# BarclayII/audiogan

Measured on AMD Instinct MI355X. Metric: audio-samples/sec per G+D train step (8 kHz, 8192-sample clips), higher is better.
Workload: dtype f32; 1 GPU; C2: full audiogan.py Conv1d/LSTM G + D, batch 64 per GPU, 8192-sample white-noise clips, frame_size 256 (T=32), canonical G+D step, adam, per-parameter clip d=1 g=0.1; global_batch=64, clip_len=8192, parallelism=dp1, launch=hipGraph replay (1 graph per step)

## Files before the change

### audiogan_amd/_lib.py

```python
import ctypes as C
import os

_HERE = os.path.dirname(os.path.abspath(__file__))
LIB_PATH = os.path.join(_HERE, 'libaudiogan_hip.so')

AG_OK, AG_ERR_ARG, AG_ERR_LAUNCH, AG_ERR_UNSUPPORTED = 0, -1, -2, -3
ACT_NONE, ACT_LEAKY, ACT_TANH, ACT_LEAKY_GATE = 0, 1, 2, 3
OPT_RMSPROP, OPT_ADAM = 0, 1
FLAG_NAN, FLAG_BIG = 1, 2

vp, i32, i64, f32 = C.c_void_p, C.c_int32, C.c_int64, C.c_float


class WnDesc(C.Structure):
    _fields_ = [('v', vp), ('g', vp), ('w', vp), ('wpa', vp), ('wpb', vp), ('inv_norm', vp),
                ('rows', i32), ('cols', i32), ('d1', i32), ('K', i32), ('stride', i32), ('pad_', i32)]


class WnBwdDesc(C.Structure):
    _fields_ = [('v', vp), ('g', vp), ('dw', vp), ('dv', vp), ('dg', vp), ('rows', i32), ('cols', i32),
                ('accumulate', i32), ('pad_', i32)]


class ConvArgs(C.Structure):
# ... 26 lines not shown
    'ag_arch': (C.c_char_p, []),
    'ag_last_error': (C.c_char_p, []),
    'ag_last_kernel': (C.c_char_p, []),
    'ag_weight_norm_fwd': (C.c_int, [vp, C.c_int, C.c_int, vp]),
    'ag_weight_norm_bwd': (C.c_int, [vp, C.c_int, C.c_int, vp]),
    'ag_conv1d_engine': (C.c_int, [C.POINTER(ConvArgs), vp]),
    'ag_prep_conv_weight': (C.c_int, [vp, vp, vp, C.c_int, C.c_int, C.c_int, C.c_int, C.c_int, vp]),
    'ag_wpa_numel': (i64, [C.c_int, C.c_int, C.c_int]),
    'ag_wpb_numel': (i64, [C.c_int, C.c_int, C.c_int, C.c_int]),
    'ag_conv1d_wgrad': (C.c_int, [vp, i64, i64, vp, i64, i64, vp] + [C.c_int] * 8 + [vp]),
    'ag_conv1d_o1_fwd': (C.c_int, [vp, i64, i64, vp, vp, vp, i64, C.c_int, C.c_int, C.c_int, C.c_int, C.c_int,
                                   C.c_int, f32, vp]),
    'ag_conv1d_o1_bwd_data': (C.c_int, [vp, i64, vp, vp, i64, i64, C.c_int, C.c_int, C.c_int, C.c_int, C.c_int,
                                        C.c_int, vp]),
    'ag_conv1d_o1_wgrad': (C.c_int, [vp, i64, vp, i64, i64, vp, C.c_int, C.c_int, C.c_int, C.c_int, C.c_int, vp]),
    'ag_channel_sum': (C.c_int, [vp, i64, i64, vp, C.c_int, C.c_int, C.c_int, C.c_int, vp]),
    'ag_lstm_front_bwd_step': (C.c_int, [vp, C.c_int, vp, C.c_int, vp, C.c_int, C.c_int, vp, vp, C.c_int, vp, vp, vp,
                                         vp, vp, vp, C.c_int, C.c_int, vp]),
    'ag_leaky_bwd': (C.c_int, [vp, i64, i64, vp, i64, i64, vp, i64, i64, vp, i64, i64, vp, vp, C.c_int,
                               C.c_int, C.c_int, f32, vp]),
    'ag_gemm': (C.c_int, [vp, C.c_int, C.c_int, vp, C.c_int, C.c_int, vp, C.c_int, C.c_int,
                          C.c_int, C.c_int, f32, f32, vp, vp, C.c_int, C.c_int, f32, vp]),
    'ag_col_sum': (C.c_int, [vp, C.c_int, C.c_int, vp, C.c_int, C.c_int, C.c_int, vp]),
    'ag_lstm_cell_fwd': (C.c_int, [vp, C.c_int, vp, C.c_int, vp, C.c_int, vp, C.c_int, vp, C.c_int,
                                   vp, C.c_int, vp, C.c_int, C.c_int, C.c_int, vp]),
    'ag_lstm_cell_bwd': (C.c_int, [vp, C.c_int, vp, C.c_int, vp, C.c_int, vp, C.c_int, vp, C.c_int,
                                   vp, C.c_int, vp, C.c_int, vp, C.c_int, vp, C.c_int, vp, C.c_int,
                                   C.c_int, C.c_int, vp]),
    'ag_gru_cell_fwd': (C.c_int, [vp, vp, vp, C.c_int, vp, C.c_int, C.c_int, C.c_int, vp]),
    'ag_gru_cell_bwd': (C.c_int, [vp, vp, vp, C.c_int, vp, C.c_int, vp, vp, vp, C.c_int, C.c_int, C.c_int, vp]),
    'ag_skinny_gemm': (C.c_int, [vp, C.c_int, vp, C.c_int, C.c_int, vp, C.c_int, C.c_int, C.c_int, C.c_int,
                                 f32, vp, C.c_int, f32, C.c_int, vp]),
    'ag_lstm_step_fwd': (C.c_int, [vp, vp, C.c_int, vp, C.c_int, C.c_int, vp, vp, vp, vp, vp, C.c_int,
                                   C.c_int, C.c_int, vp]),
    'ag_lstm_seq_fwd': (C.c_int, [vp, vp, vp, vp, vp, vp, vp, C.c_int, C.c_int, C.c_int, C.c_int, C.c_int, C.c_int, vp]),
    'ag_lstm_seq_bwd': (C.c_int, [vp, vp, vp, vp, vp, vp, vp, vp, C.c_int, C.c_int, C.c_int, C.c_int, C.c_int, C.c_int, C.c_int, vp]),
    'ag_set_precision': (C.c_int, [C.c_int]),
    'ag_get_precision': (C.c_int, []),
    'ag_bind_workspace': (C.c_int, [vp, i64]),
    'ag_conv1d_wgrad_ws_numel': (i64, [C.c_int] * 5),
    'ag_gemm_ws_numel': (i64, [C.c_int] * 4),
    'ag_skinny_ws_numel': (i64, [C.c_int] * 3),
    'ag_persist_debug': (C.c_int, [i64, C.c_int]),
    'ag_lstm_persist_ok': (C.c_int, [C.c_int, C.c_int, C.c_int, C.c_int]),
    'ag_lstm_persist_ws_bytes': (i64, [C.c_int, C.c_int, C.c_int]),
    'ag_lstm_seq_fwd_persist': (C.c_int, [vp, vp, vp, vp, C.c_int, vp, vp, vp, i64, C.c_int, C.c_int, C.c_int, C.c_int, C.c_int, vp]),
# ... 82 lines not shown
```

### audiogan_amd/csrc/gemm.hip

```cpp
#include <cstdlib>
#include <type_traits>

#include "common.h"
#include "gemm_tile.h"

#ifndef GBK
#define GBK 16
#endif
#define GKQ (GBK / 4)


template <int ROWS>
struct KContig {
  static constexpr int ITER = ROWS * (GBK / 4) / 256;
  static_assert(ITER >= 1, "tile too small");
  f32x4 v[ITER];
  __device__ __forceinline__ void load(const float* __restrict__ G, int ld, int r0, int nrows, int k0, int K,
                                       bool vec, int tid) {
#pragma unroll
    for (int it = 0; it < ITER; ++it) {
      const int idx = tid + it * 256;
      const int r = idx / GKQ, kq = idx % GKQ;
      const int gr = r0 + r, gk = k0 + kq * 4;
      f32x4 q = {0.f, 0.f, 0.f, 0.f};
// ... 642 lines not shown
extern "C" int ag_col_sum(const void* X, int x_bf16, int ldx, float* out, int M, int N, int accumulate, void* stream) {
  const AgWs ws = ag_ws_take();
  AG_REQUIRE(X && out && M > 0 && N > 0 && ldx >= N, "ag_col_sum: bad args");
  const int gx = ag_cdiv(N, 64);
  int gy = ag_cdiv(1024, gx);
  if (gy > ag_cdiv(M, 16)) gy = ag_cdiv(M, 16);
  if (gy < 1) gy = 1;
  float* part = nullptr;
  if (gy > 1 && ws.p && ws.numel >= 2 * (int64_t)N) {
    if ((int64_t)gy * N > ws.numel) gy = (int)(ws.numel / N);
    part = ws.p;
  } else {
    gy = 1;
  }
  const int rows_per = ag_cdiv(M, gy);
  gy = ag_cdiv(M, rows_per);
  if (gy == 1) part = nullptr;
  hipLaunchKernelGGL(col_sum_kernel, dim3(gx, gy), dim3(256), 0, (hipStream_t)stream, (const float*)X, ldx, out, M,
                     N, rows_per, part, accumulate, x_bf16 ? 1 : 0);
  AG_CHECK_LAUNCH("ag_col_sum");
  if (part) return ag_slab_reduce(part, gy, N, out, accumulate ? 1 : 0, (hipStream_t)stream);
  return AG_OK;
}
```

### audiogan_amd/csrc/pointwise.hip

```cpp
#include "common.h"

__global__ __launch_bounds__(256) void weight_norm_fwd_kernel(const ag_wn_desc* __restrict__ descs) {
  const ag_wn_desc d = descs[blockIdx.y];
  const int lane = threadIdx.x & 63;
  const int r = blockIdx.x * 4 + (threadIdx.x >> 6);
  if (r >= d.rows) return;
  const float* v = d.v + (int64_t)r * d.cols;
  float ss = 0.f;
  for (int i = lane; i < d.cols; i += 64) {
    const float x = v[i];
    ss += x * x;
  }
  ss = ag_wave_sum(ss);
  const float nrm = sqrtf(ss);
  const float sc = d.g[r] / nrm;
  if (lane == 0 && d.inv_norm) d.inv_norm[r] = 1.f / nrm;
  const int d0p32 = (d.rows + 31) / 32 * 32;
  const int s = d.stride > 0 ? d.stride : 1;
  const int mt = (d.K + s - 1) / s;
  const int mp = (d.d1 * s + 31) / 32 * 32;
  const bool aligned = d.wpb && ag_scatter_aligned(d.K, s, d.pad);
  unsigned short* qa = d.wpa ? reinterpret_cast<unsigned short*>(d.wpa + ag_wq_offset((d.d1 + 1) & ~1, d.K, d0p32)) : nullptr;
  unsigned short* qb = d.wpb ? reinterpret_cast<unsigned short*>(d.wpb + ag_wq_offset((d.rows + 1) & ~1, mt, mp)) : nullptr;
  for (int i = lane; i < d.cols; i += 64) {
// ... 723 lines not shown
      const int64_t o = (int64_t)b * obs + (int64_t)j * ors + i;
      const float v = tile[tx][ty + 8 * k];
      if (OUT16) reinterpret_cast<unsigned short*>(out)[o] = (unsigned short)(ag_pack_bf16(v, v) & 0xFFFFu);
      else reinterpret_cast<float*>(out)[o] = v;
    }
  }
}

extern "C" int ag_transpose_batched(const void* in, int in_bf16, int64_t ibs, int64_t irs, void* out, int out_bf16, int64_t obs,
                                    int64_t ors, int B, int R, int Cc, void* stream) {
  AG_REQUIRE(in && out && B > 0 && R > 0 && Cc > 0 && B <= 65535, "ag_transpose_batched: bad args");
  AG_REQUIRE(irs >= Cc && ors >= R, "ag_transpose_batched: a row pitch is smaller than its row");
  AG_REQUIRE(ag_cdiv(R, 32) <= 65535, "ag_transpose_batched: too many rows");
  const dim3 grid(ag_cdiv(Cc, 32), ag_cdiv(R, 32), B);
  hipStream_t st = (hipStream_t)stream;
  if (!in_bf16 && !out_bf16) hipLaunchKernelGGL((transpose_batched_kernel<false, false>), grid, dim3(256), 0, st, in, ibs, irs, out, obs, ors, R, Cc);
  if (!in_bf16 && out_bf16) hipLaunchKernelGGL((transpose_batched_kernel<false, true>), grid, dim3(256), 0, st, in, ibs, irs, out, obs, ors, R, Cc);
  if (in_bf16 && !out_bf16) hipLaunchKernelGGL((transpose_batched_kernel<true, false>), grid, dim3(256), 0, st, in, ibs, irs, out, obs, ors, R, Cc);
  if (in_bf16 && out_bf16) hipLaunchKernelGGL((transpose_batched_kernel<true, true>), grid, dim3(256), 0, st, in, ibs, irs, out, obs, ors, R, Cc);
  AG_CHECK_LAUNCH("ag_transpose_batched");
  return AG_OK;
}

__global__ __launch_bounds__(256) void build_zc_kernel(const float* __restrict__ z, const float* __restrict__ c,
                                                       float* __restrict__ zc, int B, int T, int ns, int es) {
  const int F = ns + es;
  const int64_t n = (int64_t)T * B * F;
  for (int64_t i = (int64_t)blockIdx.x * 256 + threadIdx.x; i < n; i += (int64_t)gridDim.x * 256) {
    const int j = (int)(i % F);
    const int64_t tb = i / F;
    const int b = (int)(tb % B), t = (int)(tb / B);
    zc[i] = j < ns ? z[((int64_t)b * T + t) * ns + j] : c[(int64_t)b * es + (j - ns)];
  }
}

extern "C" int ag_build_zc(const float* z, const float* c, float* zc, int B, int T, int ns, int es, void* stream) {
  AG_REQUIRE(z && c && zc && B > 0 && T > 0 && ns >= 0 && es >= 0 && ns + es > 0, "ag_build_zc: bad args");
  const int64_t n = (int64_t)T * B * (ns + es);
  int gx = (int)ag_cdiv64(n, 256 * 4);
  if (gx > 4096) gx = 4096;
  hipLaunchKernelGGL(build_zc_kernel, dim3(gx), dim3(256), 0, (hipStream_t)stream, z, c, zc, B, T, ns, es);
  AG_CHECK_LAUNCH("ag_build_zc");
  return AG_OK;
}

struct CriticBatchP {
// ... 312 lines not shown
```

### audiogan_amd/kernels.py

```python
import ctypes as C

import torch

from . import _lib
from ._lib import lib, check, ACT_NONE, ACT_LEAKY, ACT_TANH, ACT_LEAKY_GATE, OPT_RMSPROP, OPT_ADAM

LEAKY_SLOPE = 0.01


def _stream():
    return C.c_void_p(torch.cuda.current_stream().cuda_stream)


def _p(t):
    return C.c_void_p(t.data_ptr()) if t is not None else C.c_void_p(0)


def _chk(t, name, dtype=torch.float32):
    if t is None:
        return
    if not t.is_cuda:
        raise RuntimeError('audiogan_amd: %s must be a CUDA (HIP) tensor; there is no CPU path' % name)
    if t.dtype != dtype:
        raise TypeError('audiogan_amd: %s must be %s, got %s' % (name, dtype, t.dtype))
# ... 375 lines not shown
        check(lib.ag_gemm(_p(A), lda, int(ta), _p(B), ldb, int(tb), _p(Cm), ldc, M, N, K, alpha, beta,
                          _p(bias), _p(res), ldres, act, slope, _stream()), 'ag_gemm')
    finally:
        if hold:
            lib.ag_defer_reduces(3)


def col_sum(X, out, accumulate=True, defer=True):
    ldx = _mat_any(X, 'X')
    _chk(out, 'out')
    M, N = X.shape
    assert out.numel() == N and out.is_contiguous()
    hold = (not defer) and reduces_recording()
    if hold:
        lib.ag_defer_reduces(2)
    try:
        _ws = _bind_ws(min(_SMALL_WS, 64 * N) if M > 16 else 0, out.device)
        check(lib.ag_col_sum(_p(X), int(_is16(X)), ldx, _p(out), M, N, int(bool(accumulate)), _stream()), 'ag_col_sum')
    finally:
        if hold:
            lib.ag_defer_reduces(3)


def lstm_cell_fwd(gates, c_prev, c_out, h_out=None, y_out=None, h_prev=None, valid=None, t=0):
    ldg = _mat(gates, 'gates')
    B, H4 = gates.shape
    H = H4 // 4
    _chk(valid, 'valid', torch.int64)
    ld = lambda x, n: (_mat(x, n) if x is not None else 0)
    for x in (c_prev, c_out, h_out, y_out, h_prev):
        assert x is None or tuple(x.shape) == (B, H)
    check(lib.ag_lstm_cell_fwd(_p(gates), ldg, _p(c_prev), ld(c_prev, 'c_prev'), _p(h_out),
                               ld(h_out, 'h_out'), _p(c_out), ld(c_out, 'c_out'), _p(y_out),
                               ld(y_out, 'y_out'), _p(h_prev), ld(h_prev, 'h_prev'), _p(valid), t, B, H,
                               _stream()), 'ag_lstm_cell_fwd')


def lstm_cell_bwd(gates_act, c_prev, c_new, dh, dy, dc_next, dgates, dc_prev, dh_pass=None,
                  valid=None, t=0):
    B, H4 = gates_act.shape
    H = H4 // 4
    _chk(valid, 'valid', torch.int64)
    ld = lambda x, n: (_mat(x, n) if x is not None else 0)
    for x in (c_prev, c_new, dh, dy, dc_next, dc_prev, dh_pass):
        assert x is None or tuple(x.shape) == (B, H)
    assert tuple(dgates.shape) == (B, H4)
# ... 55 lines not shown


def bct_to_tbc(x, out=None, out_dtype=None):
    _chk_any(x, 'x')
    B, Cc, T = x.shape
    assert x.stride(2) == 1
    if out is None:
        out = torch.empty(T, B, Cc, device=x.device, dtype=out_dtype or x.dtype)
    _chk_any(out, 'out')
    check(lib.ag_transpose_batched(_p(x), int(_is16(x)), x.stride(0), x.stride(1), _p(out), int(_is16(out)), Cc, B * Cc, B, Cc,
                                   T, _stream()), 'ag_transpose_batched')
    return out


def tbc_to_bct(x, out=None, out_dtype=None):
    _chk_any(x, 'x')
    T, B, Cc = x.shape
    assert x.is_contiguous()
    if out is None:
        out = torch.empty(B, Cc, T, device=x.device, dtype=out_dtype or x.dtype)
    _chk_any(out, 'out')
    check(lib.ag_transpose_batched(_p(x), int(_is16(x)), Cc, B * Cc, _p(out), int(_is16(out)), Cc * T, T, B, T, Cc, _stream()),
          'ag_transpose_batched')
    return out


def rowdot_ok(x, w):
    return x.dim() == 2 and x.stride(1) == 1 and w.numel() == x.size(1) and w.is_contiguous()


def rowdot_fwd(x, w, bias, y):
    ldx = _mat_any(x, 'x')
    _chk(w, 'w'); _chk(bias, 'bias'); _chk(y, 'y')
    M, Kd = x.shape
    assert rowdot_ok(x, w) and y.numel() == M
    ldy = y.stride(0) if M > 1 else 1
    check(lib.ag_rowdot_fwd(_p(x), int(_is16(x)), ldx, _p(w), _p(bias), _p(y), ldy, M, Kd, _stream()), 'ag_rowdot_fwd')


def rowdot_bwd(dy, x, w, dx=None, dw=None, db=None, gate=False, slope=LEAKY_SLOPE, accumulate=True):
    ldx = _mat_any(x, 'x')
    _chk(dy, 'dy'); _chk(w, 'w'); _chk_any(dx, 'dx'); _chk(dw, 'dw'); _chk(db, 'db')
    M, Kd = x.shape
    assert rowdot_ok(x, w) and dy.numel() == M
    lddx = _mat_any(dx, 'dx') if dx is not None else 0
    assert dx is None or (tuple(dx.shape) == (M, Kd) and dx.dtype == x.dtype), 'x and dx share a storage type'
# ... 229 lines not shown
        nl = w_[3] if len(w_) > 3 else 1
        only = Profiler.only
        if key is None:
            sig = _call_sig(a, k)
            if only is not None and seen.get(sig, only) != only:
                return fn(*a, **k)
        elif only is not None and key != only:
            return fn(*a, **k)
        e0, e1 = torch.cuda.Event(enable_timing=True), torch.cuda.Event(enable_timing=True)
        e0.record()
        r = fn(*a, **k)
        e1.record()
        if key is None:
            key = seen[sig] = lib.ag_last_kernel().decode()
        Profiler.records.append((key, fl, by, e0, e1, nl))
        return r
    wrapped.__name__ = name
    wrapped.__doc__ = fn.__doc__
    wrapped.__module__ = __name__
    globals()[name] = wrapped


for _n, _w in (('gemm', _work_gemm), ('conv_engine', _work_conv), ('conv_wgrad', _work_wgrad),
               ('channel_sum', None), ('leaky_bwd', None), ('col_sum', None), ('lstm_cell_fwd', None),
               ('lstm_cell_bwd', None), ('weight_norm_fwd', None), ('weight_norm_bwd', None),
               ('bce_logits_fwd', None), ('bce_logits_bwd', None), ('act_fwd', None), ('act_bwd', None),
               ('axpby', None), ('grad_norms', None), ('opt_step', None)):
    _instrument(_n, _w)


def _al16(t):
    return t.data_ptr() % 16 == 0


def skinny_ok(A, B, tb):
    M, Kd = A.shape
    ok = M <= 256 and Kd % 8 == 0 and A.stride(1) == 1 and A.stride(0) % 4 == 0 and _al16(A)
    if tb:
        ok = ok and B.stride(1) == 1 and B.stride(0) % 4 == 0 and _al16(B)
    return ok


def skinny_gemm(A, B, Cm, tb=False, beta=0.0, bias=None, act=ACT_NONE, slope=LEAKY_SLOPE, atomic=False):
    lda, ldb, ldc = _mat(A, 'A'), _mat(B, 'B'), _mat(Cm, 'C')
    M, N = Cm.shape
    Kd = A.size(1)
    assert A.size(0) == M and (B.size(1) if tb else B.size(0)) == Kd and (B.size(0) if tb else B.size(1)) == N
# ... 758 lines not shown
```

### audiogan_amd/modules.py

```python
import torch
import torch.nn as nn

from . import ops
from .common import prepare_groups
from .ops import ConvSpec


def div_roundup(x, d):
    return (x + d - 1) // d


def roundup(x, d):
    return (x + d - 1) // d * d


class Replicated(nn.Module):

    def __init__(self, module):
        super().__init__()
        self.module = module

    def forward(self, *a, **k):
        return self.module(*a, **k)

# ... 252 lines not shown
            _add(self._head.group, r.linear, 'weight')
            _add(self._head.group, r.linear, 'bias')
        for i in (0, 2):
            _add(self._head.group, self.classifier.module[i], 'weight')
            _add(self._head.group, self.classifier.module[i], 'bias')

    def _stride_prods(self, dev):
        t = getattr(self, '_prods', None)
        if t is None or t[0].device != dev:
            p = torch.tensor(list(_cumprod([s for _, s, _ in self.cnn_struct])), device=dev).view(-1, 1)
            t = self._prods = (p, p - 1)
        return t

    def _rnn_weights(self, layer):
        out = []
        for suffix in ('', '_reverse'):
            for n in ('weight_ih', 'weight_hh', 'bias_ih', 'bias_hh'):
                out.append(getattr(self.rnn, '%s_l%d%s' % (n, layer, suffix)))
        return out

    def stride_products(self):
        return list(_cumprod([s for _, s, _ in self.cnn_struct]))

    def features(self, x, length, lens_all=None):
        if lens_all is None:
            length = length.to(x.device).long()
            prods, prods_m1 = self._stride_prods(x.device)
            lens_all = torch.div(length.view(1, -1) + prods_m1, prods, rounding_mode='floor')
        lens_list = [lens_all[i] for i in range(lens_all.size(0))]
        acts = ops.DConvStackFn.apply(x, self._stack, lens_list, *self._stack.group.params())
        return acts, lens_list

    def stores_bf16(self, batch, dev):
        K = ops.K
        dev = torch.device(dev)
        h = self._state_size // 2
        return bool(dev.type == 'cuda' and K.bf16_storage() and K.lstm_step_ok(batch, h) and
                    K.lstm_persist_ok(batch, h, 2, dev) and K.lstm_persist_bwd_ok(batch, h, 2, dev))

    def classify(self, a, n, c):
        ss, es = self._state_size, self._embed_size
        b, tq = a.size(0), a.size(2)
        s16 = self.stores_bf16(b, a.device)
        seq = ops.TimeMajorFn.apply(a, s16)
        for layer in range(self._num_layers):
            seq = ops.LSTMSeqFn.apply(seq, n, 2, c if layer == 0 else None, *self._rnn_weights(layer))
        logits = ops.DHeadFn.apply(seq.reshape(tq * b, ss), self._head, *self._head.group.params())
        return logits.view(tq, b).t()

    def early_params(self):
        conv = set(id(p) for p in self.cnn.parameters())
        return [p for p in self.parameters() if id(p) not in conv]

    def prepare_weights(self):
        prepare_groups([self._stack.group, self._head.group])

    def forward(self, x, length, c, percent_used=0.1, lens_all=None):
        self.prepare_weights()
        acts, lens_list = self.features(x, length, lens_all)
        n = lens_list[-1]
        return self.classify(acts[-1], n, c), list(acts), lens_list, n


class Embedder(nn.Module):

    def __init__(self, output_size=100, char_embed_size=50, num_layers=1, num_chars=256):
        super().__init__()
        self._output_size = output_size
        self._char_embed_size = char_embed_size
        self._num_layers = num_layers
        self.embed = Replicated(nn.Embedding(num_chars, char_embed_size))
        self.rnn = nn.LSTM(char_embed_size, output_size // 2, num_layers, bidirectional=True)

    def forward(self, chars, length):
        nl, b, o = self._num_layers, chars.size(0), self._output_size
        dev = self.embed.module.weight.device
        length = length.to(dev).long()
        seq = self.embed.module.weight[chars.to(dev).long()].permute(1, 0, 2).contiguous()
        for layer in range(nl):
            w = []
            for suffix in ('', '_reverse'):
                for n in ('weight_ih', 'weight_hh', 'bias_ih', 'bias_hh'):
                    w.append(getattr(self.rnn, '%s_l%d%s' % (n, layer, suffix)))
            seq = ops.LSTMSeqFn.apply(seq, length, 2, None, *w)
# ... 24 lines not shown
```

### audiogan_amd/ops.py

```python
import torch

from . import kernels as K
from .kernels import ACT_NONE, ACT_LEAKY, ACT_TANH, ACT_LEAKY_GATE

from .common import PARAM_EPOCH, Prepared, WNGroup, _zeros_like_list


class ConvSpec(object):
    __slots__ = ('kind', 'cin', 'cout', 'K', 'stride', 'pad', 'out_pad')

    def __init__(self, kind, cin, cout, K_, stride, pad, out_pad=0):
        self.kind, self.cin, self.cout, self.K, self.stride, self.pad = kind, cin, cout, K_, stride, pad
        self.out_pad = out_pad

    def out_len(self, lin):
        if self.kind == 'conv':
            return (lin + 2 * self.pad - self.K) // self.stride + 1
        return (lin - 1) * self.stride - 2 * self.pad + self.K + self.out_pad


def _o1(spec):
    return K.conv_o1_ok(spec.kind, spec.cout, spec.K, spec.stride, spec.pad)


# ... 102 lines not shown
            add = dslab[:, cin - ds.cout:cin] if cin >= ds.cout else None
            K.leaky_bwd(dout, out_v, dout, add_into=add, bias_grad=dws[4 * i + 3] if wg else None)
            hid = hids[i]
            if wg:
                conv_wgrad(ds, hid, dout, dws[4 * i + 2], None)
            dhid = torch.empty_like(hid)
            conv_bwd_data(ds, qw, dout, dhid, gate=hid)
            if wg:
                K.channel_sum(dhid, dws[4 * i + 1])
            if wg:
                conv_wgrad(cs, slab[:, :cin], dhid, dws[4 * i], None)
            conv_bwd_data(cs, pw, dhid, dslab[:, :cin], accumulate=True)


class DConvStack(object):
    def __init__(self, specs):
        self.specs = specs
        self.group = WNGroup()


class DConvStackFn(torch.autograd.Function):

    @staticmethod
    def forward(ctx, x, stack, lens_list, *params):
        B, L = x.shape
        ctx.set_materialize_grads(False)
        prep = stack.group.prepare()
        a = x.contiguous().view(B, 1, L)
        acts = []
        for i, sp in enumerate(stack.specs):
            lo = sp.out_len(a.size(2))
            y = torch.empty(B, sp.cout, lo, device=x.device)
            conv_fwd(sp, prep[2 * i], a, y, bias=prep[2 * i + 1].w, lens=lens_list[i], act=ACT_LEAKY)
            acts.append(y)
            a = y
        ctx.stack, ctx.lens_list, ctx.key = stack, lens_list, stack.group._key[1:]
        ctx.save_for_backward(x, *acts)
        return tuple(acts)

    @staticmethod
    def backward(ctx, *dacts):
        stack = ctx.stack
        x, acts = ctx.saved_tensors[0], ctx.saved_tensors[1:]
        prep = stack.group.prepare()
        assert stack.group._key[1:] == ctx.key, 'parameters changed between forward and backward'
        B, L = x.shape
        wg = any(ctx.needs_input_grad[3:])
        dws = stack.group.zero_dws() if wg else None
        n = len(stack.specs)
        d, gated = None, False
        with K.deferred_reduces():
            for i in reversed(range(n)):
                sp = stack.specs[i]
                g = dacts[i]
                if d is None:
                    if g is None:
                        continue
                    d = torch.empty_like(acts[i])
                    K.leaky_bwd(g.contiguous(), acts[i], d, lens=ctx.lens_list[i],
                                bias_grad=dws[2 * i + 1] if wg else None)
                elif not gated:
                    if g is not None:
                        K.axpby(g.contiguous(), d, 1.0, 1.0)
                    K.leaky_bwd(d, acts[i], d, lens=ctx.lens_list[i], bias_grad=dws[2 * i + 1] if wg else None)
                elif wg:
                    K.channel_sum(d, dws[2 * i + 1])
                xin = acts[i - 1] if i > 0 else x.contiguous().view(B, 1, L)
                if wg:
                    conv_wgrad(sp, xin, d, dws[2 * i], None)
                if i > 0 or ctx.needs_input_grad[0]:
                    dx = torch.empty_like(xin)
                    gated = i > 0 and dacts[i - 1] is None
                    conv_bwd_data(sp, prep[2 * i], d, dx, gate=acts[i - 1] if gated else None,
                                  lens=ctx.lens_list[i - 1] if gated else None)
                    d = dx
                else:
                    d = None
        grads = stack.group.backward(dws) if wg else [None] * (2 * len(stack.group.items))
        dx0 = d.view(B, L) if (ctx.needs_input_grad[0] and d is not None) else None
        return (dx0, None, None) + tuple(grads)


class DHead(object):

    def __init__(self, n_res):
        self.n_res = n_res
        self.group = WNGroup()


class TimeMajorFn(torch.autograd.Function):

    @staticmethod
    def forward(ctx, a, store16=False):
        if a.stride(2) != 1:
            a = a.contiguous()
        ctx.in_dtype = a.dtype
        return K.bct_to_tbc(a, out_dtype=torch.bfloat16 if store16 else None)

    @staticmethod
    def backward(ctx, g):
        return K.tbc_to_bct(g.contiguous(), out_dtype=ctx.in_dtype), None


# ... 231 lines not shown
```

### audiogan_amd/recurrent.py

```python
import torch

from . import kernels as K
from .kernels import ACT_NONE, ACT_TANH
from .common import WNGroup, _zeros_like_list, grad_target


STOPPER_ONLY = [False]


def _gh(*a, **k):
    from .ops import _gh as f
    return f(*a, **k)


def _small(A, B, Cm, tb=False, beta=0.0, bias=None, act=ACT_NONE, res=None):
    if res is None and K.skinny_ok(A, B, tb):
        K.skinny_gemm(A, B, Cm, tb=tb, beta=beta, bias=bias, act=act)
    else:
        K.gemm(A, B, Cm, tb=tb, beta=beta, bias=bias, res=res, act=act)


def _linear1(x, w, b, y):
    if K.rowdot_ok(x, w):
        K.rowdot_fwd(x, w, b, y)
# ... 155 lines not shown
                        K.gemm(dg[t], whh[d], dpass, beta=1.0)
        dx2 = torch.empty(T * B, Fx, device=dev)
        outs = []
        dstatic = torch.zeros_like(st) if need_ds else None
        if dgsums is None:
            dgsums = [None] * ndir
        for d in range(ndir):
            w_ih = w[4 * d]
            wx = w_ih[:, :Fx] if st is not None else w_ih
            dg2 = dgs[d].view(T * B, 4 * H)
            K.gemm(dg2, wx, dx2, beta=0.0 if d == 0 else 1.0)
            dgsum = dgsums[d]
            if want_sum:
                if not have_sum:
                    K.col_sum(dgs[d].view(T, B * 4 * H), dgsum.view(-1), accumulate=False, defer=False)
                if need_ds:
                    K.gemm(dgsum, w_ih[:, Fx:], dstatic, beta=1.0)
        if not wg:
            outs = [None] * (4 * ndir)
        tgs = [[grad_target(p_) for p_ in ctx.params[4 * d:4 * d + 4]] for d in range(ndir)] if wg else []
        direct_all = wg and all(t_ is not None for tg in tgs for t_ in tg)
        import contextlib
        with (K.deferred_reduces() if direct_all else contextlib.nullcontext()):
            for d in range(ndir if wg else 0):
                w_ih, w_hh = w[4 * d], w[4 * d + 1]
                dg2 = dgs[d].view(T * B, 4 * H)
                dgsum = dgsums[d]
                tg = tgs[d]
                direct = all(t_ is not None for t_ in tg)
                if direct:
                    dw_ih, dw_hh = tg[0], tg[1]
                else:
                    dw_ih = torch.zeros_like(w_ih)
                    dw_hh = torch.zeros_like(w_hh)
                K.gemm(dg2, x2, dw_ih[:, :Fx] if st is not None else dw_ih, ta=True, beta=1.0, defer=direct_all)
                if st is not None:
                    K.gemm(dgsum, st, dw_ih[:, Fx:], ta=True, beta=1.0, defer=direct_all)
                if T > 1:
                    if d == 0:
                        K.gemm(dgs[d][1:].view((T - 1) * B, 4 * H), y[:-1].view((T - 1) * B, ndir * H)[:, :H],
                               dw_hh, ta=True, beta=1.0, defer=direct_all)
                    else:
                        K.gemm(dgs[d][:-1].view((T - 1) * B, 4 * H),
                               y[1:].view((T - 1) * B, ndir * H)[:, H:2 * H], dw_hh, ta=True, beta=1.0, defer=direct_all)
                src, rows = (dgsum, B) if dgsum is not None else (dg2, T * B)
                if direct:
                    K.col_sum(src.view(rows, 4 * H), tg[2])
                    K.col_sum(src.view(rows, 4 * H), tg[3])
                    outs += [None, None, None, None]
                    continue
                db = torch.zeros(4 * H, device=dev)
                K.col_sum(src.view(rows, 4 * H), db)
                outs += [dw_ih, dw_hh, db, db.clone()]
        dx = dx2.view(T, B, Fx) if ctx.needs_input_grad[0] else None
        return (dx, None, None, dstatic) + tuple(outs)


def _lstm_backward16(ctx, dy, x2, y, lengths, st, gates_all, c_all, w):
    T, B, Fx, H = ctx.shape
    ndir = ctx.ndir
    dev = x2.device
    H4 = 4 * H
    whh = [w[4 * d + 1].contiguous() for d in range(ndir)]
    dgs = [torch.empty(T, B, H4, device=dev) for _ in range(ndir)]
    dg16 = torch.empty(T, B, ndir * H4, device=dev, dtype=torch.bfloat16)
    wg = any(ctx.needs_input_grad[4:])
    need_ds = st is not None and ctx.needs_input_grad[3]
    want_sum = st is not None and (wg or need_ds)
    dgsums = [torch.empty(B, H4, device=dev) for _ in range(ndir)] if want_sum else None
    have_sum = K.lstm_seq_bwd(gates_all, whh, c_all, dy, dgs, None, None, lengths, dgsum=dgsums,
                              dg16=[dg16[:, :, d * H4:(d + 1) * H4] for d in range(ndir)])
    assert have_sum or not want_sum
    dg2 = dg16.view(T * B, ndir * H4)
    dx2 = None
    if ctx.needs_input_grad[0]:
        dx2 = torch.empty(T * B, Fx, device=dev, dtype=torch.bfloat16)
        _gh(dg2, _wih16(w, ndir, Fx), C16=dx2)
    dstatic = torch.zeros_like(st) if need_ds else None
    for d in range(ndir if need_ds else 0):
        K.gemm(dgsums[d], w[4 * d][:, Fx:], dstatic, beta=1.0)
    outs = []
    if not wg:
        outs = [None] * (4 * ndir)
    tgs = [[grad_target(p_) for p_ in ctx.params[4 * d:4 * d + 4]] for d in range(ndir)] if wg else []
    direct_all = wg and all(t_ is not None for tg in tgs for t_ in tg)
    import contextlib
    with (K.deferred_reduces() if direct_all else contextlib.nullcontext()):
        for d in range(ndir if wg else 0):
            w_ih, w_hh = w[4 * d], w[4 * d + 1]
            tg = tgs[d]
            direct = all(t_ is not None for t_ in tg)
            dw_ih, dw_hh = (tg[0], tg[1]) if direct else (torch.zeros_like(w_ih), torch.zeros_like(w_hh))
            dgd = dg2[:, d * H4:(d + 1) * H4]
            _gh(dgd, x2, C=dw_ih[:, :Fx] if st is not None else dw_ih, ta=True, beta=1.0, defer=direct_all)
            if st is not None:
                K.gemm(dgsums[d], st, dw_ih[:, Fx:], ta=True, beta=1.0, defer=direct_all)
            if T > 1:
                y2 = y.view(T * B, ndir * H)
                if d == 0:
                    _gh(dgd[B:], y2[:(T - 1) * B, :H], C=dw_hh, ta=True, beta=1.0, defer=direct_all)
                else:
                    _gh(dgd[:(T - 1) * B], y2[B:, H:2 * H], C=dw_hh, ta=True, beta=1.0, defer=direct_all)
            src, rows = (dgsums[d], B) if want_sum else (dgs[d].view(T * B, H4), T * B)
            if direct:
                K.col_sum(src.view(rows, H4), tg[2])
                K.col_sum(src.view(rows, H4), tg[3])
                outs += [None, None, None, None]
                continue
            db = torch.zeros(H4, device=dev)
            K.col_sum(src.view(rows, H4), db)
            outs += [dw_ih, dw_hh, db, db.clone()]
    dx = dx2.view(T, B, Fx) if dx2 is not None else None
    return (dx, None, None, dstatic) + tuple(outs)


LSTMSeqFn._backward16 = staticmethod(_lstm_backward16)


def _frames_buffer(front, B, n, dev):
    ctot = getattr(front, 'slab_channels', 0)
    if ctot and ctot > 1 and torch.device(dev).type == 'cuda':
        return torch.empty(B, ctot, n, device=dev)[:, 0, :]
    return torch.empty(B, n, device=dev)


class GFront(object):

    def __init__(self, frame_size, num_layers, state_size):
        self.fs, self.nl, self.ss = frame_size, num_layers, state_size
        self.slab_channels = 0
        self.group = WNGroup()


class GFrontFn(torch.autograd.Function):
# ... 331 lines not shown
```

### include/audiogan_hip.h

```cpp
#ifndef AUDIOGAN_HIP_H
#define AUDIOGAN_HIP_H

#include <stdint.h>

#ifdef __cplusplus
extern "C" {
#endif

#define AG_OK 0
#define AG_ERR_ARG (-1)
#define AG_ERR_LAUNCH (-2)
#define AG_ERR_UNSUPPORTED (-3)

#define AG_ACT_NONE 0
#define AG_ACT_LEAKY 1
#define AG_ACT_TANH 2
#define AG_ACT_LEAKY_GATE 3

int ag_abi_version(void);
const char* ag_arch(void);
const char* ag_last_error(void);
const char* ag_last_kernel(void);

typedef struct ag_wn_desc {
// ... 59 lines not shown

int ag_conv1d_o1_fwd(const float* x, int64_t x_bs, int64_t x_cs, const float* w, const float* bias, float* y,
                     int64_t y_bs, int B, int C, int L, int K, int pad, int act, float slope, void* stream);
int ag_conv1d_o1_bwd_data(const float* dy, int64_t dy_bs, const float* w, float* dx, int64_t dx_bs,
                          int64_t dx_cs, int B, int C, int L, int K, int pad, int accumulate, void* stream);
int ag_conv1d_o1_wgrad(const float* dy, int64_t dy_bs, const float* x, int64_t x_bs, int64_t x_cs, float* dw,
                       int B, int C, int L, int K, int pad, void* stream);

int ag_channel_sum(const float* dy, int64_t bs, int64_t cs, float* db, int B, int C, int L, int accumulate,
                   void* stream);

int ag_leaky_bwd(const float* dy, int64_t dy_bs, int64_t dy_cs, const float* y, int64_t y_bs,
                 int64_t y_cs, float* dpre, int64_t dp_bs, int64_t dp_cs, float* add_into,
                 int64_t ad_bs, int64_t ad_cs, const int64_t* lens_i64, float* bias_grad, int B, int C,
                 int L, float slope, void* stream);

int ag_gemm(const float* A, int lda, int ta, const float* B, int ldb, int tb, float* C, int ldc,
            int M, int N, int K, float alpha, float beta, const float* bias, const float* res,
            int ldres, int act, float slope, void* stream);

int ag_col_sum(const void* X, int x_bf16 , int ldx, float* out, int M, int N,
               int accumulate, void* stream);

int ag_lstm_cell_fwd(float* gates, int ldg, const float* c_prev, int ldcp, float* h_out, int ldh,
                     float* c_out, int ldc, float* y_out, int ldy, const float* h_prev, int ldhp,
                     const int64_t* valid_i64, int t, int B, int H, void* stream);
int ag_lstm_cell_bwd(const float* gates_act, int ldg, const float* c_prev, int ldcp,
                     const float* c_new, int ldc, const float* dh, int lddh, const float* dy,
                     int lddy, const float* dc_next, int lddcn, float* dgates, int lddg,
                     float* dc_prev, int lddcp, float* dh_pass, int lddhp, const int64_t* valid_i64,
                     int t, int B, int H, void* stream);

int ag_gru_cell_fwd(float* gi, const float* gh, const float* h_prev, int ldhp, float* h_out, int ldh,
                    int B, int H, void* stream);
int ag_gru_cell_bwd(const float* gates_act, const float* gh, const float* h_prev, int ldhp,
                    const float* dh, int lddh, float* dgi, float* dgh, float* dh_prev, int lddhp, int B,
                    int H, void* stream);

#define AG_PREC_F32 0
#define AG_PREC_BF16 1
#define AG_PREC_F32X3 2
int ag_set_precision(int mode);
int ag_get_precision(void);

int ag_bind_workspace(float* ws, int64_t numel);
int64_t ag_conv1d_wgrad_ws_numel(int B, int A, int Lsh, int C, int K);
int64_t ag_gemm_ws_numel(int M, int N, int K, int act);

int ag_transpose_batched(const void* in, int in_bf16, int64_t ibs, int64_t irs, void* out, int out_bf16, int64_t obs,
                         int64_t ors, int B, int R, int Cc, void* stream);

int ag_rowdot_fwd(const void* x, int x_bf16, int ldx, const float* w, const float* bias, float* y, int64_t ldy, int M, int K,
                  void* stream);
int64_t ag_rowdot_bwd_ws_numel(int M, int K);
int ag_rowdot_bwd(const float* dy, int64_t lddy, const void* x, int ldx, const float* w, void* dx, int lddx, int h16, float* dw,
                  float* db, int accumulate, int M, int K, int gate, float slope, void* stream);
int ag_build_zc(const float* z, const float* c, float* zc, int B, int T, int ns, int es, void* stream);

int ag_gemm_h_ok(int M, int N, int K, int ta, int tb, int lda, int ldb);
int64_t ag_gemm_h_ws_numel(int M, int N, int K, int act, int has_c16);
int ag_gemm_h(const uint16_t* A, int lda, int ta, const uint16_t* B, int ldb, int tb, float* C, int ldc, uint16_t* C16,
              int ldc16, int M, int N, int K, float alpha, float beta, const float* bias, const float* res, int ldres,
              const uint16_t* res16, int ldres16, const uint16_t* gate16, int ldgate16, int act, float slope, void* stream);
int ag_to_bf16_2d(const float* src, int64_t ld_src, uint16_t* dst, int64_t ld_dst, int rows, int cols, void* stream);
int ag_critic_batch(const float* xa, int64_t xa_ld, const float* na, int64_t na_ld, int nA, const float* xb,
                    int64_t xb_ld, const float* nb, int64_t nb_ld, int nB, int L, float* x_out,
                    const int64_t* lenA_i64, const int64_t* lenB_i64, const int32_t* prods_host, int nl,
                    int64_t* lens_out_i64, const float* cA, const float* cB, int E, float* c_out, void* stream);

int ag_defer_reduces(int mode);
int ag_flush_reduces(void* stream);
int64_t ag_skinny_ws_numel(int M, int N, int K);

// ... 148 lines not shown
```

Before: 30.83 million audio-samples/sec.

## Fuse discriminator top transpose with leaky gate backward and batch LSTM bias sums

In f32 mode the discriminator conv stack now also emits the time-major copy of its last activation, so the separate transpose inside classify is skipped. In backward, the time-major gradient is transposed, gated by the leaky derivative, masked by length, and reduced into the bias gradient in one kernel instead of a transpose followed by leaky_bwd. LSTM bias column sums for both directions and both bias targets go through a single batched col_sum_pairs launch instead of four launches. The aim is fewer kernel launches and fewer passes over small tensors, at the cost of more special-case plumbing in autograd and extra workspace partitioning.

```diff
diff --git a/audiogan_amd/_lib.py b/audiogan_amd/_lib.py
--- a/audiogan_amd/_lib.py
+++ b/audiogan_amd/_lib.py
@@ -72,6 +72,8 @@
     'ag_gemm': (C.c_int, [vp, C.c_int, C.c_int, vp, C.c_int, C.c_int, vp, C.c_int, C.c_int,
                           C.c_int, C.c_int, f32, f32, vp, vp, C.c_int, C.c_int, f32, vp]),
     'ag_col_sum': (C.c_int, [vp, C.c_int, C.c_int, vp, C.c_int, C.c_int, C.c_int, vp]),
+    'ag_col_sum_pairs': (C.c_int, [vp, vp, C.c_int, vp, vp, vp, vp, C.c_int, C.c_int, C.c_int, vp]),
+    'ag_tbc_gate_bct': (C.c_int, [vp, vp, i64, i64, vp, i64, i64, vp, vp, C.c_int, C.c_int, C.c_int, f32, vp]),
     'ag_lstm_cell_fwd': (C.c_int, [vp, C.c_int, vp, C.c_int, vp, C.c_int, vp, C.c_int, vp, C.c_int,
                                    vp, C.c_int, vp, C.c_int, C.c_int, C.c_int, vp]),
     'ag_lstm_cell_bwd': (C.c_int, [vp, C.c_int, vp, C.c_int, vp, C.c_int, vp, C.c_int, vp, C.c_int,
diff --git a/audiogan_amd/csrc/gemm.hip b/audiogan_amd/csrc/gemm.hip
--- a/audiogan_amd/csrc/gemm.hip
+++ b/audiogan_amd/csrc/gemm.hip
@@ -688,3 +688,76 @@
   if (part) return ag_slab_reduce(part, gy, N, out, accumulate ? 1 : 0, (hipStream_t)stream);
   return AG_OK;
 }
+
+struct ColSumPairP {
+  const float* X[2];
+  float* oa[2];
+  float* ob[2];
+};
+
+__global__ __launch_bounds__(256) void col_sum_pairs_kernel(const ColSumPairP p, int ldx, int M, int N, int rows_per,
+                                                            float* __restrict__ part, int accumulate) {
+  const int z = blockIdx.z;
+  const float* __restrict__ X = z == 0 ? p.X[0] : p.X[1];
+  const int n = blockIdx.x * 64 + (threadIdx.x & 63);
+  const int sub = threadIdx.x >> 6;
+  const int mbeg = blockIdx.y * rows_per;
+  int mend = mbeg + rows_per;
+  if (mend > M) mend = M;
+  float s = 0.f;
+  if (n < N)
+    for (int m = mbeg + sub; m < mend; m += 4) s += X[(int64_t)m * ldx + n];
+  __shared__ float red[4][64];
+  red[sub][threadIdx.x & 63] = s;
+  __syncthreads();
+  if (sub == 0 && n < N) {
+    s = red[0][threadIdx.x] + red[1][threadIdx.x] + red[2][threadIdx.x] + red[3][threadIdx.x];
+    if (part) {
+      part[((int64_t)z * gridDim.y + blockIdx.y) * N + n] = s;
+    } else {
+      float* oa = z == 0 ? p.oa[0] : p.oa[1];
+      float* ob = z == 0 ? p.ob[0] : p.ob[1];
+      oa[n] = accumulate ? oa[n] + s : s;
+      ob[n] = accumulate ? ob[n] + s : s;
+    }
+  }
+}
+
+extern "C" int ag_col_sum_pairs(const float* X0, const float* X1, int ldx, float* out0a, float* out0b, float* out1a,
+                                float* out1b, int M, int N, int accumulate, void* stream) {
+  const AgWs ws = ag_ws_take();
+  AG_REQUIRE(X0 && out0a && out0b && M > 0 && N > 0 && ldx >= N, "ag_col_sum_pairs: bad args");
+  AG_REQUIRE(!X1 || (out1a && out1b), "ag_col_sum_pairs: the second source needs both of its targets");
+  const int nsrc = X1 ? 2 : 1;
+  const int64_t budget = ws.p ? ws.numel / nsrc : 0;
+  const int gx = ag_cdiv(N, 64);
+  int gy = ag_cdiv(1024, gx);
+  if (gy > ag_cdiv(M, 16)) gy = ag_cdiv(M, 16);
+  if (gy < 1) gy = 1;
+  float* part = nullptr;
+  if (gy > 1 && budget >= 2 * (int64_t)N) {
+    if ((int64_t)gy * N > budget) gy = (int)(budget / N);
+    part = ws.p;
+  } else {
+    gy = 1;
+  }
+  const int rows_per = ag_cdiv(M, gy);
+  gy = ag_cdiv(M, rows_per);
+  if (gy == 1) part = nullptr;
+  ColSumPairP p;
+  p.X[0] = X0; p.X[1] = X1;
+  p.oa[0] = out0a; p.ob[0] = out0b; p.oa[1] = out1a; p.ob[1] = out1b;
+  hipStream_t st = (hipStream_t)stream;
+  hipLaunchKernelGGL(col_sum_pairs_kernel, dim3(gx, gy, nsrc), dim3(256), 0, st, p, ldx, M, N, rows_per, part,
+                     accumulate);
+  AG_CHECK_LAUNCH("ag_col_sum_pairs");
+  if (!part) return AG_OK;
+  const int acc = accumulate ? 1 : 0;
+  for (int z = 0; z < nsrc; ++z) {
+    const float* pz = part + (int64_t)z * gy * N;
+    int rc = ag_slab_reduce(pz, gy, N, p.oa[z], acc, st);
+    if (rc == AG_OK) rc = ag_slab_reduce(pz, gy, N, p.ob[z], acc, st);
+    if (rc != AG_OK) return rc;
+  }
+  return AG_OK;
+}
diff --git a/audiogan_amd/csrc/pointwise.hip b/audiogan_amd/csrc/pointwise.hip
--- a/audiogan_amd/csrc/pointwise.hip
+++ b/audiogan_amd/csrc/pointwise.hip
@@ -769,6 +769,73 @@
   return AG_OK;
 }
 
+__global__ __launch_bounds__(256) void tbc_gate_bct_kernel(const float* __restrict__ g, const float* __restrict__ y,
+                                                           int64_t y_bs, int64_t y_cs, float* __restrict__ d, int64_t d_bs,
+                                                           int64_t d_cs, const int64_t* __restrict__ lens, int B, int C, int T,
+                                                           int bper, float slope, float* __restrict__ part) {
+  __shared__ float tile[32][33];
+  const int t0 = blockIdx.x * 32, c0 = blockIdx.y * 32;
+  const int tx = threadIdx.x & 31, ty = threadIdx.x >> 5;
+  float bsum[4] = {0.f, 0.f, 0.f, 0.f};
+  const int bend = min(B, (int)(blockIdx.z + 1) * bper);
+  for (int b = blockIdx.z * bper; b < bend; ++b) {
+    const int64_t lenb = lens ? lens[b] : (int64_t)1 << 60;
+#pragma unroll
+    for (int k = 0; k < 4; ++k) {
+      const int t = t0 + ty + 8 * k, c = c0 + tx;
+      tile[ty + 8 * k][tx] = (t < T && c < C) ? g[((int64_t)t * B + b) * C + c] : 0.f;
+    }
+    __syncthreads();
+#pragma unroll
+    for (int k = 0; k < 4; ++k) {
+      const int c = c0 + ty + 8 * k, t = t0 + tx;
+      if (c < C && t < T) {
+        float v = tile[tx][ty + 8 * k];
+        v = (y[(int64_t)b * y_bs + (int64_t)c * y_cs + t] > 0.f) ? v : v * slope;
+        if (t >= lenb) v = 0.f;
+        d[(int64_t)b * d_bs + (int64_t)c * d_cs + t] = v;
+        bsum[k] += v;
+      }
+    }
+    __syncthreads();
+  }
+  if (part) {
+#pragma unroll
+    for (int k = 0; k < 4; ++k) {
+      float s = bsum[k];
+#pragma unroll
+      for (int o = 16; o > 0; o >>= 1) s += __shfl_xor(s, o, 64);
+      const int c = c0 + ty + 8 * k;
+      if (tx == 0 && c < C) part[(int64_t)(blockIdx.z * gridDim.x + blockIdx.x) * C + c] = s;
+    }
+  }
+}
+
+extern "C" int ag_tbc_gate_bct(const float* g, const float* y, int64_t y_bs, int64_t y_cs, float* d, int64_t d_bs, int64_t d_cs,
+                               const int64_t* lens_i64, float* bias_grad, int B, int C, int T, float slope, void* stream) {
+  const AgWs ws = ag_ws_take();
+  AG_REQUIRE(g && y && d && B > 0 && C > 0 && T > 0, "ag_tbc_gate_bct: bad args");
+  AG_REQUIRE(y_cs >= T && d_cs >= T, "ag_tbc_gate_bct: a row pitch is smaller than its row");
+  const int gx = ag_cdiv(T, 32), gy = ag_cdiv(C, 32);
+  AG_REQUIRE(gy <= 65535 && B <= 65535, "ag_tbc_gate_bct: B or C too large");
+  int bper = (int)(((int64_t)gx * gy * B) / 2048);
+  if (bper < 1) bper = 1;
+  if (bper > B) bper = B;
+  float* part = nullptr;
+  if (bias_grad) {
+    AG_REQUIRE(ws.p && ws.numel >= (int64_t)gx * C, "%s: this reduction spans several workgroups and needs a workspace of >= %lld floats bound with ag_bind_workspace (sums are two-stage, in a fixed order; there is no float-atomic accumulation)", "ag_tbc_gate_bct", (long long)gx * C);
+    const int64_t zmax = ws.numel / ((int64_t)gx * C);
+    if (ag_cdiv(B, bper) > zmax) bper = ag_cdiv(B, (int)zmax);
+    part = ws.p;
+  }
+  const int gz = ag_cdiv(B, bper);
+  hipLaunchKernelGGL(tbc_gate_bct_kernel, dim3(gx, gy, gz), dim3(256), 0, (hipStream_t)stream, g, y, y_bs, y_cs, d, d_bs, d_cs,
+                     lens_i64, B, C, T, bper, slope, part);
+  AG_CHECK_LAUNCH("ag_tbc_gate_bct");
+  if (part) return ag_slab_reduce(part, gx * gz, C, bias_grad, 1, (hipStream_t)stream);
+  return AG_OK;
+}
+
 __global__ __launch_bounds__(256) void build_zc_kernel(const float* __restrict__ z, const float* __restrict__ c,
                                                        float* __restrict__ zc, int B, int T, int ns, int es) {
   const int F = ns + es;
diff --git a/audiogan_amd/kernels.py b/audiogan_amd/kernels.py
--- a/audiogan_amd/kernels.py
+++ b/audiogan_amd/kernels.py
@@ -421,6 +421,27 @@
             lib.ag_defer_reduces(3)
 
 
+def col_sum_pairs(pairs, accumulate=True):
+    assert 1 <= len(pairs) <= 2
+    X0 = pairs[0][0]
+    if not X0.is_cuda:
+        for X, oa, ob in pairs:
+            col_sum(X, oa, accumulate=accumulate)
+            col_sum(X, ob, accumulate=accumulate)
+        return
+    ldx = _mat(X0, 'X')
+    M, N = X0.shape
+    for X, oa, ob in pairs:
+        assert tuple(X.shape) == (M, N) and _mat(X, 'X') == ldx
+        for o in (oa, ob):
+            _chk(o, 'out')
+            assert o.numel() == N and o.is_contiguous()
+    second = pairs[1] if len(pairs) > 1 else (None, None, None)
+    _ws = _bind_ws(len(pairs) * min(_SMALL_WS, 64 * N) if M > 16 else 0, X0.device)
+    check(lib.ag_col_sum_pairs(_p(X0), _p(second[0]), ldx, _p(pairs[0][1]), _p(pairs[0][2]), _p(second[1]), _p(second[2]),
+                               M, N, int(bool(accumulate)), _stream()), 'ag_col_sum_pairs')
+
+
 def lstm_cell_fwd(gates, c_prev, c_out, h_out=None, y_out=None, h_prev=None, valid=None, t=0):
     ldg = _mat(gates, 'gates')
     B, H4 = gates.shape
@@ -522,6 +543,29 @@
     _chk_any(out, 'out')
     check(lib.ag_transpose_batched(_p(x), int(_is16(x)), Cc, B * Cc, _p(out), int(_is16(out)), Cc * T, T, B, T, Cc, _stream()),
           'ag_transpose_batched')
+    return out
+
+
+def tbc_gate_bct(g, y, lens=None, slope=LEAKY_SLOPE, bias_grad=None, out=None):
+    if not g.is_cuda:
+        out = tbc_to_bct(g, out=out)
+        leaky_bwd(out, y, out, lens=lens, slope=slope, bias_grad=bias_grad)
+        return out
+    _chk(g, 'g')
+    T, B, Cc = g.shape
+    assert g.is_contiguous() and tuple(y.shape) == (B, Cc, T)
+    ys = _bcl(y, 'y')
+    _chk(lens, 'lens', torch.int64)
+    if out is None:
+        out = torch.empty(B, Cc, T, device=g.device)
+    os_ = _bcl(out, 'out')
+    assert tuple(out.shape) == (B, Cc, T)
+    if bias_grad is not None:
+        _chk(bias_grad, 'bias_grad')
+        assert bias_grad.is_contiguous() and bias_grad.numel() == Cc
+        _ws = _bind_ws(min(_SMALL_WS, B * ((T + 31) // 32) * Cc), bias_grad.device)
+    check(lib.ag_tbc_gate_bct(_p(g), _p(y), ys[0], ys[1], _p(out), os_[0], os_[1], _p(lens), _p(bias_grad), B, Cc, T, slope,
+                              _stream()), 'ag_tbc_gate_bct')
     return out
 
 
@@ -797,7 +841,8 @@
 
 
 for _n, _w in (('gemm', _work_gemm), ('conv_engine', _work_conv), ('conv_wgrad', _work_wgrad),
-               ('channel_sum', None), ('leaky_bwd', None), ('col_sum', None), ('lstm_cell_fwd', None),
+               ('channel_sum', None), ('leaky_bwd', None), ('col_sum', None), ('col_sum_pairs', None),
+               ('tbc_gate_bct', None), ('lstm_cell_fwd', None),
                ('lstm_cell_bwd', None), ('weight_norm_fwd', None), ('weight_norm_bwd', None),
                ('bce_logits_fwd', None), ('bce_logits_bwd', None), ('act_fwd', None), ('act_bwd', None),
                ('axpby', None), ('grad_norms', None), ('opt_step', None)):
diff --git a/audiogan_amd/modules.py b/audiogan_amd/modules.py
--- a/audiogan_amd/modules.py
+++ b/audiogan_amd/modules.py
@@ -298,13 +298,15 @@
     def stride_products(self):
         return list(_cumprod([s for _, s, _ in self.cnn_struct]))
 
-    def features(self, x, length, lens_all=None):
+    def features(self, x, length, lens_all=None, time_major=False):
         if lens_all is None:
             length = length.to(x.device).long()
             prods, prods_m1 = self._stride_prods(x.device)
             lens_all = torch.div(length.view(1, -1) + prods_m1, prods, rounding_mode='floor')
         lens_list = [lens_all[i] for i in range(lens_all.size(0))]
-        acts = ops.DConvStackFn.apply(x, self._stack, lens_list, *self._stack.group.params())
+        acts = ops.DConvStackFn.apply(x, self._stack, lens_list, time_major, *self._stack.group.params())
+        if time_major:
+            return acts[:-1], lens_list, acts[-1]
         return acts, lens_list
 
     def stores_bf16(self, batch, dev):
@@ -314,11 +316,12 @@
         return bool(dev.type == 'cuda' and K.bf16_storage() and K.lstm_step_ok(batch, h) and
                     K.lstm_persist_ok(batch, h, 2, dev) and K.lstm_persist_bwd_ok(batch, h, 2, dev))
 
-    def classify(self, a, n, c):
+    def classify(self, a, n, c, seq=None):
         ss, es = self._state_size, self._embed_size
         b, tq = a.size(0), a.size(2)
         s16 = self.stores_bf16(b, a.device)
-        seq = ops.TimeMajorFn.apply(a, s16)
+        if seq is None or s16:
+            seq = ops.TimeMajorFn.apply(a, s16)
         for layer in range(self._num_layers):
             seq = ops.LSTMSeqFn.apply(seq, n, 2, c if layer == 0 else None, *self._rnn_weights(layer))
         logits = ops.DHeadFn.apply(seq.reshape(tq * b, ss), self._head, *self._head.group.params())
@@ -333,9 +336,13 @@
 
     def forward(self, x, length, c, percent_used=0.1, lens_all=None):
         self.prepare_weights()
-        acts, lens_list = self.features(x, length, lens_all)
+        seq = None
+        if ops.K.get_precision() != 'bf16':
+            acts, lens_list, seq = self.features(x, length, lens_all, time_major=True)
+        else:
+            acts, lens_list = self.features(x, length, lens_all)
         n = lens_list[-1]
-        return self.classify(acts[-1], n, c), list(acts), lens_list, n
+        return self.classify(acts[-1], n, c, seq), list(acts), lens_list, n
 
 
 class Embedder(nn.Module):
diff --git a/audiogan_amd/ops.py b/audiogan_amd/ops.py
--- a/audiogan_amd/ops.py
+++ b/audiogan_amd/ops.py
@@ -148,7 +148,7 @@
 class DConvStackFn(torch.autograd.Function):
 
     @staticmethod
-    def forward(ctx, x, stack, lens_list, *params):
+    def forward(ctx, x, stack, lens_list, time_major, *params):
         B, L = x.shape
         ctx.set_materialize_grads(False)
         prep = stack.group.prepare()
@@ -162,6 +162,9 @@
             a = y
         ctx.stack, ctx.lens_list, ctx.key = stack, lens_list, stack.group._key[1:]
         ctx.save_for_backward(x, *acts)
+        ctx.time_major = bool(time_major)
+        if time_major:
+            return tuple(acts) + (K.bct_to_tbc(acts[-1]),)
         return tuple(acts)
 
     @staticmethod
@@ -171,15 +174,26 @@
         prep = stack.group.prepare()
         assert stack.group._key[1:] == ctx.key, 'parameters changed between forward and backward'
         B, L = x.shape
-        wg = any(ctx.needs_input_grad[3:])
+        wg = any(ctx.needs_input_grad[4:])
         dws = stack.group.zero_dws() if wg else None
         n = len(stack.specs)
+        dacts = list(dacts)
+        dseq = dacts.pop() if ctx.time_major else None
         d, gated = None, False
         with K.deferred_reduces():
+            if dseq is not None and dacts[n - 1] is None:
+                d = K.tbc_gate_bct(dseq.contiguous(), acts[n - 1], lens=ctx.lens_list[n - 1],
+                                   bias_grad=dws[2 * n - 1] if wg else None)
+                gated = True
+            elif dseq is not None:
+                dacts[n - 1] = dacts[n - 1] + K.tbc_to_bct(dseq.contiguous())
+            fused_top = d is not None
             for i in reversed(range(n)):
                 sp = stack.specs[i]
                 g = dacts[i]
-                if d is None:
+                if fused_top and i == n - 1:
+                    pass
+                elif d is None:
                     if g is None:
                         continue
                     d = torch.empty_like(acts[i])
@@ -204,7 +218,7 @@
                     d = None
         grads = stack.group.backward(dws) if wg else [None] * (2 * len(stack.group.items))
         dx0 = d.view(B, L) if (ctx.needs_input_grad[0] and d is not None) else None
-        return (dx0, None, None) + tuple(grads)
+        return (dx0, None, None, None) + tuple(grads)
 
 
 class DHead(object):
diff --git a/audiogan_amd/recurrent.py b/audiogan_amd/recurrent.py
--- a/audiogan_amd/recurrent.py
+++ b/audiogan_amd/recurrent.py
@@ -201,6 +201,7 @@
         direct_all = wg and all(t_ is not None for tg in tgs for t_ in tg)
         import contextlib
         with (K.deferred_reduces() if direct_all else contextlib.nullcontext()):
+            bias_pairs = []
             for d in range(ndir if wg else 0):
                 w_ih, w_hh = w[4 * d], w[4 * d + 1]
                 dg2 = dgs[d].view(T * B, 4 * H)
@@ -224,13 +225,14 @@
                                y[1:].view((T - 1) * B, ndir * H)[:, H:2 * H], dw_hh, ta=True, beta=1.0, defer=direct_all)
                 src, rows = (dgsum, B) if dgsum is not None else (dg2, T * B)
                 if direct:
-                    K.col_sum(src.view(rows, 4 * H), tg[2])
-                    K.col_sum(src.view(rows, 4 * H), tg[3])
+                    bias_pairs.append((src.view(rows, 4 * H), tg[2], tg[3]))
                     outs += [None, None, None, None]
                     continue
                 db = torch.zeros(4 * H, device=dev)
                 K.col_sum(src.view(rows, 4 * H), db)
                 outs += [dw_ih, dw_hh, db, db.clone()]
+            if bias_pairs:
+                K.col_sum_pairs(bias_pairs)
         dx = dx2.view(T, B, Fx) if ctx.needs_input_grad[0] else None
         return (dx, None, None, dstatic) + tuple(outs)
 
@@ -265,6 +267,7 @@
     direct_all = wg and all(t_ is not None for tg in tgs for t_ in tg)
     import contextlib
     with (K.deferred_reduces() if direct_all else contextlib.nullcontext()):
+        bias_pairs = []
         for d in range(ndir if wg else 0):
             w_ih, w_hh = w[4 * d], w[4 * d + 1]
             tg = tgs[d]
@@ -282,13 +285,14 @@
                     _gh(dgd[:(T - 1) * B], y2[B:, H:2 * H], C=dw_hh, ta=True, beta=1.0, defer=direct_all)
             src, rows = (dgsums[d], B) if want_sum else (dgs[d].view(T * B, H4), T * B)
             if direct:
-                K.col_sum(src.view(rows, H4), tg[2])
-                K.col_sum(src.view(rows, H4), tg[3])
+                bias_pairs.append((src.view(rows, H4), tg[2], tg[3]))
                 outs += [None, None, None, None]
                 continue
             db = torch.zeros(H4, device=dev)
             K.col_sum(src.view(rows, H4), db)
             outs += [dw_ih, dw_hh, db, db.clone()]
+        if bias_pairs:
+            K.col_sum_pairs(bias_pairs)
     dx = dx2.view(T, B, Fx) if dx2 is not None else None
     return (dx, None, None, dstatic) + tuple(outs)
 
diff --git a/include/audiogan_hip.h b/include/audiogan_hip.h
--- a/include/audiogan_hip.h
+++ b/include/audiogan_hip.h
@@ -105,6 +105,9 @@
 int ag_col_sum(const void* X, int x_bf16 , int ldx, float* out, int M, int N,
                int accumulate, void* stream);
 
+int ag_col_sum_pairs(const float* X0, const float* X1, int ldx, float* out0a, float* out0b, float* out1a, float* out1b,
+                     int M, int N, int accumulate, void* stream);
+
 int ag_lstm_cell_fwd(float* gates, int ldg, const float* c_prev, int ldcp, float* h_out, int ldh,
                      float* c_out, int ldc, float* y_out, int ldy, const float* h_prev, int ldhp,
                      const int64_t* valid_i64, int t, int B, int H, void* stream);
@@ -132,6 +135,9 @@
 
 int ag_transpose_batched(const void* in, int in_bf16, int64_t ibs, int64_t irs, void* out, int out_bf16, int64_t obs,
                          int64_t ors, int B, int R, int Cc, void* stream);
+
+int ag_tbc_gate_bct(const float* g, const float* y, int64_t y_bs, int64_t y_cs, float* d, int64_t d_bs, int64_t d_cs,
+                    const int64_t* lens_i64, float* bias_grad, int B, int C, int T, float slope, void* stream);
 
 int ag_rowdot_fwd(const void* x, int x_bf16, int ldx, const float* w, const float* bias, float* y, int64_t ldy, int M, int K,
                   void* stream);
```

Result: no change. 30.93 million audio-samples/sec, median of 6 (+0.3%).
